# mjmj531/isaacgym

Measured on AMD Instinct MI355X. Metric: env-steps/sec at N_envs=16384 (1/2/4/8 GPUs) + achieved HBM GB/s vs roofline, higher is better.
Workload: dtype f32; 1 GPU; humanoid_pingpong 3-actor tilt (HumanoidPingpongTiltG1), num_envs=16384 per GPU, random U(-1,1) actions, 2 physics substeps per step, fused step kernel; variant=TT, kind=step, num_envs_per_gpu=16384, global_envs=16384, horizon_stats_every=32, prewarm_launches=512, full=False, launch=HIP graph of 32 steps, replayed, parallelism=env-shard x1, no data-path collective

## Files before the change

__graft_entry__.py:

```python
import os
import sys

ROOT = os.path.dirname(os.path.abspath(__file__))
if ROOT not in sys.path:
    sys.path.insert(0, ROOT)


def build():
    from isaacgym_amd import _lib
    _lib.build(force=False)
    from oracle import binding as oracle_binding
    oracle_binding.build()
    sys.path.insert(0, os.path.join(ROOT, "tests"))
    import shim_binding
    shim_binding.lib()
    import dr_shim_binding
    dr_shim_binding.lib()
    import play_shim_binding
    play_shim_binding.lib()
    import play_pair_shim_binding
    play_pair_shim_binding.lib()
    import play_act_shim_binding
    play_act_shim_binding.lib()
    import play_delay_shim_binding
    play_delay_shim_binding.lib()
    import train_delay_shim_binding
    train_delay_shim_binding.lib()
    import ppo_meter_shim_binding
    ppo_meter_shim_binding.lib()
    import render_shim_binding
    render_shim_binding.lib()
    import render_aa_shim_binding
    render_aa_shim_binding.lib()
    import ta_outcome_shim_binding
    ta_outcome_shim_binding.lib()
    import serve_shim_binding
    serve_shim_binding.lib()
    import serve_curric_shim_binding
    serve_curric_shim_binding.lib()
    import urdf_assets
    urdf_assets.build_second_arm_library()
    urdf_assets.build_second_ta_library()
    import isaacgym_amd
    L = _lib.lib()
    from isaacgym_amd import scene
    assert L.ppenv_abi_version() == scene.ABI_VERSION


def smoke():
    import numpy as np
    import torch
    from isaacgym_amd import _lib, scene
    from isaacgym_amd.env import PPEnv
    from oracle import binding as oracle_binding
    sys.path.insert(0, os.path.join(ROOT, "tests"))
    import helpers

    assert torch.cuda.is_available(), "smoke() needs the GPU box"
    _lib.lib()
    n = 256
    cfg = scene.build_config("TT", num_envs=n, seed=1)
    env = PPEnv(scene.build_config("TT", num_envs=n, seed=1), device="cuda:0")
    ora = oracle_binding.OracleEnv(cfg)
    probe = helpers.SensitivityProbe(oracle_binding, cfg)
    oa, ra = helpers.obs_atol(), helpers.reward_atol(cfg)
    rng = np.random.default_rng(0)
    excluded = 0
    for t in range(8):
        a = rng.uniform(-1, 1, (n, 7)).astype(np.float32)
        st = ora.get_state()
        env.set_state(st)
        ora.step(a)
        env.step(torch.from_numpy(a).cuda())
        torch.cuda.synchronize()
        keep = ~probe.sensitive(st, a, ora)
        excluded += int((~keep).sum())
        assert np.array_equal(env.reset_buf.cpu().numpy()[keep], ora.reset_buf[keep])
        helpers.assert_close(env.obs_buf.cpu().numpy()[keep], ora.obs_buf[keep], f"smoke: obs, step {t}", atol=oa)
        helpers.assert_close(env.rew_buf.cpu().numpy()[keep], ora.rew_buf[keep], f"smoke: rew, step {t}", atol=ra)
    assert excluded <= 4, excluded
    assert env.status == 0
    env.close()
    print(f"smoke ok: fused HIP step matches the CPU oracle on {n} envs x 8 steps (rtol 1e-4, the tests' atol; {excluded} env-steps on a switch set aside)")


if __name__ == "__main__":
    build()
    if len(sys.argv) > 1 and sys.argv[1] == "smoke":
        smoke()
```

isaacgym_amd/csrc/ppenv.hip:

```cpp
#include <hip/hip_runtime.h>

#include <algorithm>
#include <cstdio>
#include <cstdlib>
#include <cstring>
#include <new>

using std::min;
using std::max;

#if defined(PP_STAMP)
__device__ unsigned long long pp_stamp_buf[4096 * 32];
#endif
#include "ppenv_device.h"
#include "ppenv_host.h"

using namespace pp;

namespace {

constexpr int kBlock = 64;
constexpr int kObsStride = PPENV_NUM_OBS + 1;
constexpr int kMaxSplitSubsteps = 4;

// ... 354 lines not shown
        return;
    }

    PP_STAMP_AT(16);
    constexpr int EB = kBlock / BW;
    const int bw = wave - A;
    const int env = bw * EB + lane;
    const int bi = base + env;
    const bool bactive = lane < EB && bi < n;
    EnvStateT<A> st;
    float rew[A], pre_vx = 0.f;
    long long reset = 0;
    V3 next_serve = mk(0, 0, 0);
    ArmGeom<T::kShapes> g[A];
    V3 bound[A];
    float qs[A * ND], qds[A * ND];
    EnvDR bdr;
    uint32_t bdr_ep0 = 0;
#pragma unroll
    for (int a = 0; a < A; a++) rew[a] = 0.f;
    if (bactive) {
        if (!G) {
#pragma unroll
            for (int d = 0; d < A * ND; d++) { qs[d] = b.dof_pos[(size_t)d * n + bi]; qds[d] = b.dof_vel[(size_t)d * n + bi]; }
        }
        float bl[13];
#pragma unroll
        for (int k = 0; k < 13; k++) bl[k] = b.ball[(size_t)k * n + bi];
        st.ball.p = mk(bl[0], bl[1], bl[2]);
#pragma unroll
        for (int k = 0; k < 4; k++) st.ball.quat[k] = bl[3 + k];
        st.ball.v = mk(bl[7], bl[8], bl[9]);
        st.ball.w = mk(bl[10], bl[11], bl[12]);
        st.progress = b.progress[(size_t)bi * A];
#pragma unroll
        for (int a = 0; a < A; a++) st.flags[a] = b.flags[(size_t)a * n + bi];
        st.episode = b.episode[bi];
        pre_vx = st.ball.v.x;
#pragma unroll
        for (int a = 0; a < A; a++) { static_geometry<T>(K.site[a], g[a]); bound[a] = ld3(K.site[a].bound_center); }
        if (DR) {
            bdr.es = drt.es ? drt.es[bi] : 1.f;
            bdr.fs = drt.fs ? drt.fs[bi] : 1.f;
            bdr.obs_sigma = drt.obs_sigma;
            bdr.key_progress = (uint32_t)st.progress;
            bdr_ep0 = st.episode;
        }
    }
    PP_STAMP_AT(17);
    for (int s = 0; s < substeps; s++) {
        if (G) {
#pragma unroll
            for (int a = 0; a < A; a++) PP_AWAIT(&s_gflag[a], s + 1);
        } else if (s > 0) {
#pragma unroll
            for (int a = 0; a < A; a++) PP_AWAIT(&s_flag[a], s);
            if (bactive) {
#pragma unroll
                for (int a = 0; a < A; a++)
#pragma unroll
                    for (int d = 0; d < ND; d++) { qs[a * ND + d] = s_q[s - 1][a * 2 * ND + d][env]; qds[a * ND + d] = s_q[s - 1][a * 2 * ND + ND + d][env]; }
            }
        }
        PP_STAMP_AT(18 + 2 * s);
        if (bactive) {
#pragma unroll
            for (int a = 0; a < A; a++) {
                if (G) {
                    MovingGeom<T>::each(g[a], [&](int k, float& v) { v = s_geom[s & 1][a][k][env]; });
                } else {
                    JointSave js[ND];
                    GeomVisitor<T> gv(g[a]);
                    fk_sweep<T>(K.site[a], &qs[a * ND], &qds[a * ND], js, gv);
                }
            }
            PP_STAMP_AT(25);
            ball_substep<T, A, DR>(K, st.ball, g, bound, &bdr);
        }
        if (G) publish(&s_bflag, s + 1);
        PP_STAMP_AT(19 + 2 * s);
    }
#pragma unroll
    for (int a = 0; a < A; a++) PP_AWAIT(&s_flag[a], substeps + 1);
    if (bactive) {
        BodyState bodies[A * NB];
        LdsRowStore stores[A];
#pragma unroll
        for (int a = 0; a < A; a++) {
#pragma unroll
            for (int d = 0; d < ND; d++) {
                st.q[a * ND + d] = s_q[substeps - 1][a * 2 * ND + d][env];
                st.qd[a * ND + d] = s_q[substeps - 1][a * 2 * ND + ND + d][env];
                st.dof_force[a * ND + d] = s_tau[a * ND + d][env];
            }
            static_body<false>(K.site[a], bodies[a * NB]);
            bodies[a * NB + NB - 1].pos = mk(s_paddle[a * 3 + 0][env], s_paddle[a * 3 + 1][env], s_paddle[a * 3 + 2][env]);
            stores[a].row = &s_obs[(a * kBlock + env) * kObsStride];
        }
        next_serve = mk(s_serve[0][env], s_serve[1][env], s_serve[2][env]);
        if (DR && drt.obs_sigma > 0.f) {
            NoisyRowStore nstores[A];
#pragma unroll
            for (int a = 0; a < A; a++)
                nstores[a] = NoisyRowStore{stores[a].row, bdr.obs_sigma, K.seed, (uint32_t)(K.env_id_offset + bi), bdr_ep0, bdr.key_progress, 16u + (uint32_t)(a * PPENV_NUM_OBS)};
            post_physics_env<A, false>(K, (uint32_t)(K.env_id_offset + bi), st, bodies, pre_vx, &next_serve, rew, reset, nstores);
        } else
            post_physics_env<A, false>(K, (uint32_t)(K.env_id_offset + bi), st, bodies, pre_vx, &next_serve, rew, reset, stores);
        s_reset[env] = (int)reset;
    }
    publish(&s_flag_ball, 1);
    PP_STAMP_AT(22);
    __builtin_amdgcn_wave_barrier();
    PP_STAMP_AT(23);
#pragma unroll
    for (int a = 0; a < A; a++)
        flush_obs_cols<6 * NB, PPENV_NUM_OBS>(s_obs, b.obs, a * kBlock + bw * EB, BW == 1 ? nvalid : max(0, min(EB, nvalid - bw * EB)),
                                              (size_t)(base + bw * EB) * A + a, A, lane);
    if (bactive) {
        if (kBallStoresDofs) {
#pragma unroll
            for (int d = 0; d < A * ND; d++) {
                st_state(&b.dof_pos[(size_t)d * n + bi], st.q[d]);
                st_state(&b.dof_vel[(size_t)d * n + bi], st.qd[d]);
                st_state(&b.dof_force[(size_t)d * n + bi], st.dof_force[d]);
            }
        }
        store_ball(b, n, bi, st.ball);
        store_task<A>(b, n, bi, st, rew, reset);
    }
    PP_STAMP_AT(24);
}

template <class T, int A>
__global__ __launch_bounds__(kBlock) void init_kernel(const StepConsts K, DevBuffers b, int mode, int serve_on) {
    __shared__ float s_obs[A * kBlock * kObsStride];
    const int n = K.num_envs;
    const int base = blockIdx.x * kBlock;
    const int lane = threadIdx.x;
    const int i = base + lane;
    const int nvalid = min(kBlock, n - base);
    if (i < n) {
        EnvStateT<A> st;
        st.episode = mode == 0 ? 0u : b.episode[i] + 1u;
        V3 serve = serve_on ? mk(b.serve[i], b.serve[(size_t)n + i], b.serve[2 * (size_t)n + i])
                            : serve_velocity(K, (uint32_t)(K.env_id_offset + i), st.episode);
        reset_state(K, st, serve, true);
#pragma unroll
        for (int d = 0; d < A * ND; d++) st.dof_force[d] = 0.f;
        st.progress = 0;
        float rew[A];
#pragma unroll
        for (int a = 0; a < A; a++) {
            st.flags[a] = PPENV_FLAG_NO_BOUNCE;
            rew[a] = 0.f;
            BodyState bodies[NB];
            bodies_of_state<T>(K.site[a], &st.q[a * ND], &st.qd[a * ND], bodies);
            V3 bpos[NB], bvel[NB];
#pragma unroll
            for (int j = 0; j < NB; j++) { bpos[j] = bodies[j].pos; bvel[j] = bodies[j].lin; }
            LdsRowStore store{&s_obs[(a * kBlock + lane) * kObsStride]};
            write_obs(bpos, bvel, K.site[a].hinv, &st.q[a * ND], &st.qd[a * ND], st.ball.p, st.ball.v, store);
        }
        store_state<A>(b, n, i, st, rew, 1);
    }
    __syncthreads();
#pragma unroll
// ... 662 lines not shown
```

isaacgym_amd/csrc/ppenv_device.h:

```cpp
#pragma once

#include <math.h>
#include <stddef.h>
#include <stdint.h>
#include <string.h>

#include "../../include/ppenv.h"

#if defined(__HIPCC__)
#define PP_HD __host__ __device__ __forceinline__
#else
#define PP_HD inline __attribute__((always_inline))
#endif

#if defined(PP_STAMP) && defined(__HIP_DEVICE_COMPILE__)
#define PP_STAMP_AT(k)                                                                      \
    do {                                                                                    \
        __builtin_amdgcn_sched_barrier(0);                                                  \
        unsigned long long t_;                                                              \
        asm volatile("s_memtime %0\n\ts_waitcnt lgkmcnt(0)" : "=s"(t_) : : "memory");      \
        __builtin_amdgcn_sched_barrier(0);                                                  \
        if ((threadIdx.x & 63) == 0) pp_stamp_buf[blockIdx.x * 32 + (k)] = t_;                      \
    } while (0)
extern __device__ unsigned long long pp_stamp_buf[];
// ... 224 lines not shown
    float sa, ca, sz, cz;
    sincos_small(tilt_deg * deg, sa, ca);
    sincos_small(tilt_z_deg * deg, sz, cz);
    if (form == PPENV_VARIANT_T3) return mk(-speed * ca, -speed * sa, 0.f);
    if (form == PPENV_VARIANT_TT || form == PPENV_VARIANT_T4) return mk(-speed * ca * cz, -speed * sa * sz, -speed * sa);
    return mk(-speed * ca * cz, speed * sa * cz, speed * sz);
}
PP_HD V3 serve_velocity(const StepConsts& K, uint32_t gid, uint32_t episode) {
    float u0 = rng_uniform(K.seed, gid, episode, 0);
    float u1 = rng_uniform(K.seed, gid, episode, 1);
    float u2 = rng_uniform(K.seed, gid, episode, 2);
    float speed = K.serve_speed_lo + (K.serve_speed_hi - K.serve_speed_lo) * u0;
    float a = K.serve_tilt_lo_deg + (K.serve_tilt_hi_deg - K.serve_tilt_lo_deg) * u1;
    float az = K.serve_tilt_z_lo_deg + (K.serve_tilt_z_hi_deg - K.serve_tilt_z_lo_deg) * u2;
    return serve_from_draws(K.rc.variant, speed, a, az);
}
PP_HD float pd_target(float action, float lo, float hi, float clip) {
    const float a = fminf(fmaxf(action, -clip), clip);
    return 0.5f * (hi + lo) + 0.5f * (hi - lo) * a;
}

struct EnvDR {
    float kp[PPENV_NUM_DOF], kd[PPENV_NUM_DOF], ms[PPENV_NUM_DOF];
    float es, fs;
    float act_sigma, obs_sigma;
    uint32_t key_progress;
};
PP_HD void dr_gauss_pair(uint64_t seed, uint32_t gid, uint32_t episode, uint32_t progress, uint32_t pair, float& g_cos, float& g_sin) {
    const uint32_t k = progress * 256u + 2u * pair;
    const float u1 = rng_uniform(seed ^ 0x5DEECE66Dull, gid, episode, 2u * k), u2 = rng_uniform(seed ^ 0x5DEECE66Dull, gid, episode, 2u * k + 1u);
#if defined(__HIP_DEVICE_COMPILE__)
    const float rad = __builtin_amdgcn_sqrtf(-1.3862944f * __builtin_amdgcn_logf(fmaxf(u1, 5.9604645e-8f)));
    g_cos = rad * __builtin_amdgcn_cosf(u2);
    g_sin = rad * __builtin_amdgcn_sinf(u2);
#else
    const float rad = sqrtf(-2.0f * logf(fmaxf(u1, 5.9604645e-8f)));
    g_cos = rad * cosf(6.2831853f * u2);
    g_sin = rad * sinf(6.2831853f * u2);
#endif
}
PP_HD float dr_gauss(uint64_t seed, uint32_t gid, uint32_t episode, uint32_t progress, uint32_t index) {
    float c, s;
    dr_gauss_pair(seed, gid, episode, progress, index >> 1, c, s);
    return (index & 1u) ? s : c;
}

struct JointKin { float origin_xyz[3]; float origin_rot[9]; };
struct JointDrive { float lower, upper, kp, kd, effort, vel_limit, armature; };
struct JointInertial { float mass; float com[3]; float inertia[6]; };
struct ModelShape { float a[3], b[3]; float radius; };
struct ModelPaddle { float center[3], normal[3]; float radius, half_thickness; };


template <int NSHAPES>
struct ArmGeom {
    V3 pc, pn, vpc, pnd;
    V3 a[NSHAPES], b[NSHAPES];
    V3 va[NSHAPES], vb[NSHAPES];
};

struct JointSave {
    float c, s;
    V3 w, v;
    V3 ua, ub;
    float dinv, u;
};

struct BodyState { V3 pos; M3 rot; V3 lin, ang; };

template <class T, class Visitor>
PP_HD void fk_sweep(const ArmSite& S, const float* q, const float* qd, JointSave* js, Visitor& vis) {
    M3 Rp = ldm(S.base_rot);
    V3 pp = ld3(S.base_pos);
    V3 wp = mk(0, 0, 0), vp = mk(0, 0, 0);
#pragma unroll
    for (int i = 0; i < ND; i++) {
        const JointKin J = T::kin(i);
        float s, c;
        sincos_joint(q[i], s, c);
        M3 E = T::axis(i) == 0 ? joint_rot<0>(J.origin_rot, c, s) : (T::axis(i) == 1 ? joint_rot<1>(J.origin_rot, c, s) : joint_rot<2>(J.origin_rot, c, s));
        V3 r = ld3(J.origin_xyz);
        V3 pw = pp + mul(Rp, r);
        M3 Rw = mul(Rp, E);
        V3 w = tmul(E, wp);
        V3 v = tmul(E, vp + cross(wp, r));
        if (T::axis(i) == 0) w.x += qd[i]; else if (T::axis(i) == 1) w.y += qd[i]; else w.z += qd[i];
        js[i].c = c; js[i].s = s; js[i].w = w; js[i].v = v;
        vis(i, Rw, pw, w, v);
        Rp = Rw; pp = pw; wp = w; vp = v;
    }
}

template <class T>
struct GeomVisitor {
    ArmGeom<T::kShapes>& g;
    PP_HD explicit GeomVisitor(ArmGeom<T::kShapes>& gg) : g(gg) {}
    PP_HD void operator()(int i, const M3& Rw, V3 pw, V3 w, V3 v) {
        const V3 ww = mul(Rw, w), vw = mul(Rw, v);
        if (i == ND - 1) {
            const ModelPaddle P = T::paddle();
            V3 off = mul(Rw, ld3(P.center));
            g.pc = pw + off;
            g.vpc = vw + cross(ww, off);
            g.pn = mul(Rw, ld3(P.normal));
            g.pnd = cross(ww, g.pn);
        }
#pragma unroll
        for (int s = 0; s < T::kShapes; s++)
            if (T::shape_link(s) == i) {
                const ModelShape sh = T::shape(s);
                V3 oa = mul(Rw, ld3(sh.a)), ob = mul(Rw, ld3(sh.b));
                g.a[s] = pw + oa; g.va[s] = vw + cross(ww, oa);
                g.b[s] = pw + ob; g.vb[s] = vw + cross(ww, ob);
            }
    }
};
template <class T>
PP_HD void static_geometry(const ArmSite& S, ArmGeom<T::kShapes>& g) {
#pragma unroll
    for (int s = 0; s < T::kShapes; s++)
        if (T::shape_link(s) < 0) { g.a[s] = ld3(S.static_a[s]); g.b[s] = ld3(S.static_b[s]); g.va[s] = mk(0, 0, 0); g.vb[s] = mk(0, 0, 0); }
}

template <class T, bool FULL>
struct BodyVisitor {
    ArmGeom<T::kShapes>& g;
    BodyState* bodies;
    PP_HD BodyVisitor(ArmGeom<T::kShapes>& gg, BodyState* b) : g(gg), bodies(b) {}
    PP_HD void operator()(int i, const M3& Rw, V3 pw, V3 w, V3 v) {
        GeomVisitor<T> gv(g);
        gv(i, Rw, pw, w, v);
        V3 ww = mul(Rw, w), vw = mul(Rw, v);
        bodies[1 + i].pos = pw; bodies[1 + i].lin = vw;
        if (FULL) { bodies[1 + i].rot = Rw; bodies[1 + i].ang = ww; }
        if (i == ND - 1) {
#pragma unroll
            for (int j = 8; j < NB; j++) {
                const JointKin f = T::tip_frame(j);
                V3 off = mul(Rw, ld3(f.origin_xyz));
                bodies[j].pos = pw + off;
                bodies[j].lin = vw + cross(ww, off);
                if (FULL) { bodies[j].rot = mul(Rw, ldm(f.origin_rot)); bodies[j].ang = ww; }
            }
        }
    }
};
template <bool FULL>
PP_HD void static_body(const ArmSite& S, BodyState& b) {
    b.pos = ld3(S.root_pos); b.lin = mk(0, 0, 0);
    if (FULL) { b.rot = ldm(S.root_rot); b.ang = mk(0, 0, 0); }
}

template <class T, bool DR = false>
PP_HD void aba_solve(const ArmSite& S, JointSave* js, const float* qd, const float* tau, const float* arm_eff, float* qdd, const EnvDR* dr = nullptr) {
    S3 cA = {0, 0, 0, 0, 0, 0}, cD = {0, 0, 0, 0, 0, 0};
    M3 cB = {{0, 0, 0, 0, 0, 0, 0, 0, 0}};
    V3 cn = mk(0, 0, 0), cf = mk(0, 0, 0);
#pragma unroll
    for (int i = ND - 1; i >= 0; i--) {
        const JointKin JK = T::kin(i);
        const JointInertial J = T::inertial(i);
        const int ax = T::axis(i);
        V3 w = js[i].w, v = js[i].v;
        const float msc = DR ? dr->ms[i] : 1.f;
        float m = DR ? J.mass * msc : J.mass;
        V3 cm = ld3(J.com);
        V3 mc = cm * m;
        float cc = dot(cm, cm);
        float Jin[6];
#pragma unroll
        for (int t = 0; t < 6; t++) Jin[t] = DR ? J.inertia[t] * msc : J.inertia[t];
        S3 A = {Jin[0] + m * (cc - cm.x * cm.x), Jin[1] + m * (cc - cm.y * cm.y), Jin[2] + m * (cc - cm.z * cm.z),
                Jin[3] - m * cm.x * cm.y, Jin[4] - m * cm.x * cm.z, Jin[5] - m * cm.y * cm.z};
        V3 h_ang = mul(A, w) + cross(mc, v);
        V3 h_lin = v * m - cross(mc, w);
        V3 pn = cross(w, h_ang) + cross(v, h_lin) + cn;
        V3 pf = cross(w, h_lin) + cf;
        add_sym(A, cA);
        M3 B = {{cB.m[0], cB.m[1] - mc.z, cB.m[2] + mc.y, cB.m[3] + mc.z, cB.m[4], cB.m[5] - mc.x, cB.m[6] - mc.y, cB.m[7] + mc.x, cB.m[8]}};
        S3 D = {cD.xx + m, cD.yy + m, cD.zz + m, cD.xy, cD.xz, cD.yz};

        V3 ua = symcol(A, ax), ub = row(B, ax);
        float dinv = rcp_fast(symdiag(A, ax) + arm_eff[i]);
        float u = tau[i] - comp(pn, ax);
        js[i].ua = ua; js[i].ub = ub; js[i].dinv = dinv; js[i].u = u;
        if (i > 0) {
            sym_rank1_sub(A, ua, dinv);
            sym_rank1_sub(D, ub, dinv);
            V3 uad = ua * dinv;
#pragma unroll
            for (int r = 0; r < 3; r++) {
                float k = comp(uad, r);
                B.m[3 * r] -= k * ub.x; B.m[3 * r + 1] -= k * ub.y; B.m[3 * r + 2] -= k * ub.z;
            }
            V3 e = unit(ax);
            V3 cw = cross(w, e) * qd[i], cv = cross(v, e) * qd[i];
            float ud = u * dinv;
            V3 pan = pn + mul(A, cw) + mul(B, cv) + ua * ud;
            V3 paf = pf + tmul(B, cw) + mul(D, cv) + ub * ud;
            M3 E = ax == 0 ? joint_rot<0>(JK.origin_rot, js[i].c, js[i].s) : (ax == 1 ? joint_rot<1>(JK.origin_rot, js[i].c, js[i].s) : joint_rot<2>(JK.origin_rot, js[i].c, js[i].s));
            V3 r = ld3(JK.origin_xyz);
            S3 Ar = rot_sym(E, A), Dr = rot_sym(E, D);
            M3 Br = mul_t(mul(E, B), E);
            V3 nr = mul(E, pan), fr = mul(E, paf);
            M3 Dm = from_sym(Dr);
            M3 Bp;
#pragma unroll
            for (int j = 0; j < 3; j++) {
                V3 x = cross(r, col(Dm, j));
                Bp.m[j] = Br.m[j] + x.x; Bp.m[3 + j] = Br.m[3 + j] + x.y; Bp.m[6 + j] = Br.m[6 + j] + x.z;
            }
            V3 wp0 = cross(r, row(Bp, 0)), wp1 = cross(r, row(Bp, 1)), wp2 = cross(r, row(Bp, 2));
            V3 wb0 = cross(r, row(Br, 0)), wb1 = cross(r, row(Br, 1)), wb2 = cross(r, row(Br, 2));
            cA.xx = Ar.xx + wp0.x + wb0.x; cA.yy = Ar.yy + wp1.y + wb1.y; cA.zz = Ar.zz + wp2.z + wb2.z;
            cA.xy = Ar.xy + wp1.x + wb0.y; cA.xz = Ar.xz + wp2.x + wb0.z; cA.yz = Ar.yz + wp2.y + wb1.z;
            cB = Bp; cD = Dr;
            cn = nr + cross(r, fr); cf = fr;
        }
    }
    V3 aw = mk(0, 0, 0);
    V3 av = ld3(S.base_grav);
#pragma unroll
    for (int i = 0; i < ND; i++) {
        const JointKin J = T::kin(i);
        const int ax = T::axis(i);
        M3 E = ax == 0 ? joint_rot<0>(J.origin_rot, js[i].c, js[i].s) : (ax == 1 ? joint_rot<1>(J.origin_rot, js[i].c, js[i].s) : joint_rot<2>(J.origin_rot, js[i].c, js[i].s));
        V3 r = ld3(J.origin_xyz);
        V3 e = unit(ax);
        V3 aw2 = tmul(E, aw) + cross(js[i].w, e) * qd[i];
        V3 av2 = tmul(E, av + cross(aw, r)) + cross(js[i].v, e) * qd[i];
        float a = (js[i].u - dot(js[i].ua, aw2) - dot(js[i].ub, av2)) * js[i].dinv;
        qdd[i] = a;
        if (ax == 0) aw2.x += a; else if (ax == 1) aw2.y += a; else aw2.z += a;
        aw = aw2; av = av2;
    }
}

template <class T, bool DR = false>
PP_HD void arm_substep(const ArmSite& S, JointSave* js, float* q, float* qd, const float* target, float h, float* tau_drive, const EnvDR* dr = nullptr) {
    float tau[ND], arm[ND], qdd[ND];
#pragma unroll
    for (int d = 0; d < ND; d++) {
        const JointDrive J = T::drive(d);
        const float kp = DR ? J.kp * dr->kp[d] : J.kp, kd = DR ? J.kd * dr->kd[d] : J.kd;
        float err = target[d] - q[d];
        tau[d] = fminf(fmaxf(kp * (err - h * qd[d]) - kd * qd[d], -J.effort), J.effort);
        arm[d] = J.armature + h * kd + h * h * kp;
    }
    aba_solve<T, DR>(S, js, qd, tau, arm, qdd, dr);
#pragma unroll
    for (int d = 0; d < ND; d++) {
        const JointDrive J = T::drive(d);
        const float kp = DR ? J.kp * dr->kp[d] : J.kp, kd = DR ? J.kd * dr->kd[d] : J.kd;
        float err = target[d] - q[d];
        float vn = qd[d] + h * qdd[d];
        tau_drive[d] = fminf(fmaxf(kp * (err - h * vn) - kd * vn, -J.effort), J.effort);
        vn = fminf(fmaxf(vn, -J.vel_limit), J.vel_limit);
        float qn = q[d] + h * vn;
        if (qn > J.upper) { qn = J.upper; vn = fminf(vn, 0.f); }
        if (qn < J.lower) { qn = J.lower; vn = fmaxf(vn, 0.f); }
        q[d] = qn; qd[d] = vn;
    }
}

struct Ball { V3 p, v, w; float quat[4]; };

struct BallConsts {
    float contact_offset, bounce_threshold, depen_cap, r;
    float inv_kr;
    float stick_factor;
};

PP_HD void contact_resolve(const BallConsts& k, Ball& b, V3 n, float s, V3 u, float e, float mu) {
    if (!(s < k.contact_offset)) return;
    V3 vrel = b.v + cross(b.w, n * (-k.r)) - u;
    float vn = dot(vrel, n);
    if (vn < 0.f) {
        float e_eff = (-vn > k.bounce_threshold) ? e : 0.f;
        float jn = -(1.f + e_eff) * vn;
        V3 vt = vrel - n * vn;
        float vt2 = dot(vt, vt);
        if (vt2 > 1e-18f) {
            float inv = rsq_fast(vt2);
            V3 dir = vt * inv;
            float jt = fminf(mu * jn, vt2 * inv * k.stick_factor);
            b.v = b.v - dir * jt;
            b.w = b.w + cross(n, dir) * (jt * k.inv_kr);
        }
        b.v = b.v + n * jn;
    }
    if (s < 0.f) b.p = madd(b.p, n, fminf(-s, k.depen_cap));
}
PP_HD float clampf(float x, float lo, float hi) { return fminf(fmaxf(x, lo), hi); }

PP_HD void contact_box(const BallConsts& k, Ball& b, const ppenv_box& box) {
    V3 d = b.p - ld3(box.center);
    V3 h = ld3(box.half);
    float reach = k.r + k.contact_offset;
// ... 80 lines not shown
    V3 sc0[A][T::kShapes], svc[A][T::kShapes];
    float sr2[A][T::kShapes];
#pragma unroll
    for (int arm = 0; arm < A; arm++)
#pragma unroll
        for (int s = 0; s < T::kShapes; s++) {
            sc0[arm][s] = (g[arm].a[s] + g[arm].b[s]) * 0.5f;
            svc[arm][s] = (g[arm].va[s] + g[arm].vb[s]) * 0.5f;
            V3 hl = (g[arm].b[s] - g[arm].a[s]) * 0.5f;
            float rr = sqrtf(dot(hl, hl)) + T::shape(s).radius + reach;
            sr2[arm][s] = rr * rr;
        }
    PP_STAMP_AT(26);
    for (int m = 0; m < M; m++) {
        const float t = (float)m * hb;
        PP_STAMP_AT(27 + (m & 3));
        b.v.z += gdv;
        b.w = b.w * damp;
        contact_resolve(k, b, mk(0, 0, 1), b.p.z - ground_z - k.r, mk(0, 0, 0), ground_e, ground_mu);
        contact_box(k, b, table);
        contact_box(k, b, net);
#pragma unroll
        for (int arm = 0; arm < A; arm++) {
            const ArmGeom<T::kShapes>& ga = g[arm];
            V3 db = b.p - bound[arm];
            if (dot(db, db) < K.bound_r2) {
                V3 cc = madd(ga.pc, ga.vpc, t);
                V3 dpc = b.p - cc;
                if (dot(dpc, dpc) < pad_r2) {
                    V3 nn = madd(ga.pn, ga.pnd, t);
                    nn = nn * rsq_fast(dot(nn, nn));
                    contact_disc(k, b, cc, nn, ga.vpc, ga.pnd, P.radius, P.half_thickness, pad_e, pad_mu);
                }
#pragma unroll
                for (int s = 0; s < T::kShapes; s++) {
                    V3 dsc = b.p - madd(sc0[arm][s], svc[arm][s], t);
                    if (dot(dsc, dsc) < sr2[arm][s]) {
                        const float radius = T::shape(s).radius;
                        const float e = DR ? fminf(K.shape_e[s] * dr->es, e_cap) : K.shape_e[s], mu = DR ? K.shape_mu[s] * dr->fs : K.shape_mu[s];
                        if (T::shape_link(s) < 0)
                            contact_capsule(k, b, ga.a[s], ga.b[s], mk(0, 0, 0), mk(0, 0, 0), radius, e, mu);
                        else
                            contact_capsule(k, b, madd(ga.a[s], ga.va[s], t), madd(ga.b[s], ga.vb[s], t), ga.va[s], ga.vb[s], radius, e, mu);
                    }
                }
            }
        }
        b.p = madd(b.p, b.v, hb);
    }
    PP_STAMP_AT(31);
    float wx = b.w.x, wy = b.w.y, wz = b.w.z, x = b.quat[0], y = b.quat[1], z = b.quat[2], w = b.quat[3];
    float kq = 0.5f * h;
    float nx = x + kq * (wx * w + wy * z - wz * y);
    float ny = y + kq * (wy * w + wz * x - wx * z);
    float nz = z + kq * (wz * w + wx * y - wy * x);
    float nw = w + kq * (-wx * x - wy * y - wz * z);
    float inv = rsq_fast(nx * nx + ny * ny + nz * nz + nw * nw);
    b.quat[0] = nx * inv; b.quat[1] = ny * inv; b.quat[2] = nz * inv; b.quat[3] = nw * inv;
}

PP_HD V3 quat_rotate(const float q[4], V3 v) {
    float qw = q[3];
    V3 qv = mk(q[0], q[1], q[2]);
    float s = 2.0f * (qw * qw) - 1.0f;
    V3 cr = cross(qv, v);
    float d = dot(qv, v);
    return mk(v.x * s + cr.x * qw * 2.0f + qv.x * d * 2.0f, v.y * s + cr.y * qw * 2.0f + qv.y * d * 2.0f,
              v.z * s + cr.z * qw * 2.0f + qv.z * d * 2.0f);
}
PP_HD void heading_quat_inv(const float q[4], float out[4]) {
    V3 rd = quat_rotate(q, mk(1, 0, 0));
    float heading = atan2f(rd.y, rd.x);
    float theta = (-heading) / 2.0f;
    float sz = sinf(theta), w = cosf(theta);
    float nrm = fmaxf(sqrtf(sz * sz + w * w), 1e-9f);
    out[0] = 0.f; out[1] = 0.f; out[2] = sz / nrm; out[3] = w / nrm;
}

PP_HD V3 heading_rotate(const float hinv[4], V3 v) {
    float qw = hinv[3], sz = hinv[2];
    float s = 2.0f * (qw * qw) - 1.0f;
    float k = sz * qw * 2.0f;
    return mk(v.x * s - v.y * k, v.y * s + v.x * k, v.z);
}

struct RewardIn {
    float humanoid_x;
    V3 paddle;
    float pre_vx;
    V3 bp;
    float vx;
    float power;
    long long progress;
};

PP_HD float compute_reward(const RewardConsts& c, const RewardIn& in, uint32_t& flags, long long& reset) {
    const float Bx = in.bp.x, By = in.bp.y, Bz = in.bp.z, vx = in.vx, pre_vx = in.pre_vx;
    const float alpha = c.alpha, penalty = c.penalty, threshold = 0.1f;
    const float power_reward = -c.power_coefficient * in.power;
    const int variant = c.variant;
    uint32_t f = flags;
    float reward;
    long long die = 0;
    if (variant == PPENV_VARIANT_T3) {
        V3 dp = in.paddle - in.bp;
        float dist = sqrtf(dp.x * dp.x + dp.y * dp.y + dp.z * dp.z);
        float pos_reward = 1.0f / (1.0f + 1.5f * dist * dist);
        float vel_reward = (pre_vx < 0.f && vx > 0.f) ? alpha * fabsf(vx) : 0.f;
        reward = pos_reward + power_reward + vel_reward;
        bool missed = Bx < in.paddle.x - 1e-3f;
        if (missed) { reward = reward + penalty; die = 1; }
        if (Bz < threshold) die = 1;
    } else if (variant == PPENV_VARIANT_TT || variant == PPENV_VARIANT_T4) {
        V3 dp = in.paddle - in.bp;
        float dist = sqrtf(dp.x * dp.x + dp.y * dp.y + dp.z * dp.z);
        float pos_reward = 1.0f / (1.0f + 1.5f * dist * dist);
        bool cond = pre_vx < 0.f && vx > 0.f;
        float vel_reward = (cond && !(f & PPENV_FLAG_COND_CALC)) ? alpha * fabsf(vx) : 0.f;
        if (cond) f |= PPENV_FLAG_COND_CALC;
        bool missed = Bx < in.humanoid_x - 0.05f;
        reward = missed ? 0.f + penalty : 0.f;
        bool bounce = Bz < 0.83f && vx > 0.f && By < 0.6f && By > -0.6f;
        float hit = 0.f;
        bool early = Bx < 2.44f && bounce;
        if (early && !(f & PPENV_FLAG_REWARD_CALC)) hit = c.not_hit_table_penalty;
        if (early) { f |= PPENV_FLAG_REWARD_CALC; f &= ~PPENV_FLAG_NO_BOUNCE; }
        bool inx = Bx > 2.44f && Bx < 3.1f;
        bool good = inx && bounce && (f & PPENV_FLAG_NO_BOUNCE);
        if (good && !(f & PPENV_FLAG_REWARD_CALC)) hit = c.hit_table_reward;
        if (good) f |= PPENV_FLAG_REWARD_CALC;
        if (Bx >= 3.1f && vx > 0.f && !(f & PPENV_FLAG_REWARD_CALC)) hit = c.not_hit_table_penalty;
        if (Bx >= 3.1f) f |= PPENV_FLAG_REWARD_CALC;
        float net = (Bx > 1.7f && Bx < 1.8f && vx > 0.f && By < 0.4f && By > -0.4f && Bz > 0.98f && Bz < 1.14f) ? 400.f : 0.f;
        reward += (((pos_reward + power_reward) + vel_reward) + hit) + net;
        if (Bz < threshold) die = 1;
    } else {
        bool hit_paddle = pre_vx < 0.f && vx > 1.0f;
        bool missed = (Bx < in.humanoid_x - 0.05f) || (Bx < in.paddle.x - 0.1f);
        reward = (!(f & PPENV_FLAG_MISSED_CALC) && missed) ? 0.f + penalty : 0.f;
        if (missed) f |= PPENV_FLAG_MISSED_CALC;
        float dy = in.paddle.y - By, dz = in.paddle.z - Bz;
        float dist = sqrtf(dy * dy + dz * dz);
        float pos_reward = 0.f;
        if (!(f & PPENV_FLAG_COND_CALC) || (Bx < in.humanoid_x - 0.05f)) pos_reward = 1.0f * expf(-20.0f * dist * dist);
        float vel_reward = (hit_paddle && !(f & PPENV_FLAG_COND_CALC)) ? alpha * fabsf(vx) : 0.f;
        if (hit_paddle) f |= PPENV_FLAG_COND_CALC;
        reward += (pos_reward + power_reward) + vel_reward;
        if (Bz < threshold) reward = -800.f + reward;
    }
    flags = f;
    reset = (in.progress >= (long long)c.max_episode_length - 1) ? 1 : die;
    return reward;
}

PP_HD float compute_reward_side2(const RewardConsts& c, const RewardIn& in, uint32_t& flags, long long& reset) {
    const float Bx = in.bp.x, By = in.bp.y, Bz = in.bp.z, vx = in.vx, pre_vx = in.pre_vx;
    uint32_t f = flags;
    V3 dp = in.paddle - in.bp;
    float dist = sqrtf(dp.x * dp.x + dp.y * dp.y + dp.z * dp.z);
    float pos_reward = 1.0f / (1.0f + 1.5f * dist * dist);
    bool cond = pre_vx > 0.f && vx < 0.f;
    float vel_reward = (cond && !(f & PPENV_FLAG_COND_CALC)) ? c.alpha * fabsf(vx) : 0.f;
    if (cond) f |= PPENV_FLAG_COND_CALC;
    bool missed = Bx > in.humanoid_x + 0.05f;
    float reward = missed ? 0.f + c.penalty : 0.f;
    bool bounce = Bz < 0.83f && vx < 0.f && By < 0.6f && By > -0.6f;
// ... 17 lines not shown

template <int A>
struct EnvStateT {
    float q[A * ND], qd[A * ND], dof_force[A * ND];
    Ball ball;
    long long progress;
    uint32_t flags[A], episode;
};
using EnvState = EnvStateT<1>;

template <class T, int A, bool DR = false>
PP_HD void simulate_env(const StepConsts& K, const float* actions, EnvStateT<A>& st, BodyState* bodies, float& pre_vx, const EnvDR* dr = nullptr, uint32_t gid = 0) {
    float target[A * ND];
#pragma unroll
    for (int d = 0; d < A * ND; d++) {
        float act = actions[d];
        if (DR) { if (dr->act_sigma > 0.f) act += dr->act_sigma * dr_gauss(K.seed, gid, st.episode, dr->key_progress, (uint32_t)d); }
        target[d] = pd_target(act, T::drive(d % ND).lower, T::drive(d % ND).upper, K.clip_actions);
    }
    pre_vx = st.ball.v.x;
    const int substeps = K.substeps;
    const float h = K.h;
    JointSave js[A][ND];
    ArmGeom<T::kShapes> g[A];
    V3 bound[A];
#pragma unroll
    for (int a = 0; a < A; a++) {
        bound[a] = ld3(K.site[a].bound_center);
        static_geometry<T>(K.site[a], g[a]);
        GeomVisitor<T> gv(g[a]);
        fk_sweep<T>(K.site[a], &st.q[a * ND], &st.qd[a * ND], js[a], gv);
    }
    PP_STAMP_AT(2);
    for (int s = 0; s < substeps; s++) {
        ball_substep<T, A, DR>(K, st.ball, g, bound, dr);
        PP_STAMP_AT(3 + 3 * s);
#pragma unroll
        for (int a = 0; a < A; a++)
            arm_substep<T, DR>(K.site[a], js[a], &st.q[a * ND], &st.qd[a * ND], &target[a * ND], h, &st.dof_force[a * ND], dr);
        PP_STAMP_AT(4 + 3 * s);
#pragma unroll
        for (int a = 0; a < A; a++) {
            if (s + 1 < substeps) {
                GeomVisitor<T> gv(g[a]);
                fk_sweep<T>(K.site[a], &st.q[a * ND], &st.qd[a * ND], js[a], gv);
            } else {
                BodyVisitor<T, false> bv(g[a], &bodies[a * NB]);
                fk_sweep<T>(K.site[a], &st.q[a * ND], &st.qd[a * ND], js[a], bv);
            }
        }
        PP_STAMP_AT(5 + 3 * s);
    }
#pragma unroll
    for (int a = 0; a < A; a++) static_body<false>(K.site[a], bodies[a * NB]);
}

template <class T>
PP_HD void bodies_of_state(const ArmSite& S, const float* q, const float* qd, BodyState* bodies) {
    JointSave js[ND];
    ArmGeom<T::kShapes> g;
    BodyVisitor<T, true> bv(g, bodies);
    fk_sweep<T>(S, q, qd, js, bv);
    static_body<true>(S, bodies[0]);
}

template <int A>
PP_HD void reset_state(const StepConsts& K, EnvStateT<A>& st, V3 serve, bool reset_dofs) {
    st.ball.p = ld3(K.ball_init_pos);
#pragma unroll
    for (int k = 0; k < 4; k++) st.ball.quat[k] = K.ball_init_quat[k];
    st.ball.v = serve;
    st.ball.w = mk(0, 0, 0);
    if (reset_dofs) {
#pragma unroll
        for (int d = 0; d < A * ND; d++) { st.q[d] = K.init_dof_pos[d % ND]; st.qd[d] = K.init_dof_vel[d % ND]; }
    }
}

template <int J0 = 0, int J1 = NB, class Store>
PP_HD void write_obs_bodies(const V3* body_pos, const V3* body_vel, const float hinv[4], Store& store) {
    V3 root = body_pos[0];
#pragma unroll
    for (int j = J0; j < J1; j++) {
        V3 lp = heading_rotate(hinv, body_pos[j] - root);
        V3 lv = heading_rotate(hinv, body_vel[j]);
        store(3 * j, lp.x); store(3 * j + 1, lp.y); store(3 * j + 2, lp.z);
        store(3 * NB + 3 * j, lv.x); store(3 * NB + 3 * j + 1, lv.y); store(3 * NB + 3 * j + 2, lv.z);
    }
}
template <class Store>
PP_HD void write_obs_tail(V3 root, const float hinv[4], const float* q, const float* qd, V3 ball_p, V3 ball_v, Store& store) {
#pragma unroll
    for (int d = 0; d < ND; d++) {
        store(6 * NB + d, q[d]);
        store(6 * NB + ND + d, qd[d] * 0.1f);
    }
    V3 lb = heading_rotate(hinv, ball_p - root);
    V3 lbv = heading_rotate(hinv, ball_v);
    store(6 * NB + 2 * ND, lb.x); store(6 * NB + 2 * ND + 1, lb.y); store(6 * NB + 2 * ND + 2, lb.z);
    store(6 * NB + 2 * ND + 3, lbv.x); store(6 * NB + 2 * ND + 4, lbv.y); store(6 * NB + 2 * ND + 5, lbv.z);
}
template <class Store>
PP_HD void write_obs(const V3* body_pos, const V3* body_vel, const float hinv[4], const float* q, const float* qd,
                     V3 ball_p, V3 ball_v, Store& store) {
    write_obs_bodies(body_pos, body_vel, hinv, store);
    write_obs_tail(body_pos[0], hinv, q, qd, ball_p, ball_v, store);
}

template <int A, bool BODY_OBS = true, class Store>
PP_HD void post_physics_env(const StepConsts& K, uint32_t gid, EnvStateT<A>& st, const BodyState* bodies, float pre_vx,
                            const V3* serve_override, float* rew, long long& reset, Store* stores) {
    st.progress += 1;
    RewardIn in;
    in.humanoid_x = K.site[0].root_pos[0];
    in.paddle = bodies[NB - 1].pos;
    in.pre_vx = pre_vx;
    in.bp = st.ball.p;
    in.vx = st.ball.v.x;
    float power = 0.f;
#pragma unroll
    for (int d = 0; d < A * ND; d++) power += fabsf(st.dof_force[d] * st.qd[d]);
    in.power = power;
    in.progress = st.progress;
    rew[0] = compute_reward(K.rc, in, st.flags[0], reset);
    if (A > 1) {
        RewardIn in2 = in;
        in2.humanoid_x = K.site[A - 1].root_pos[0];
        in2.paddle = bodies[(A - 1) * NB + NB - 1].pos;
        long long reset2;
        rew[A - 1] = compute_reward_side2(K.rc, in2, st.flags[A - 1], reset2);
        reset = (reset | reset2) ? 1 : 0;
    }
    if (reset) {
        st.episode += 1;
        V3 serve = serve_override ? *serve_override : serve_velocity(K, gid, st.episode);
        reset_state(K, st, serve, K.rc.variant != PPENV_VARIANT_TN);
        st.progress = 0;
#pragma unroll
        for (int a = 0; a < A; a++) st.flags[a] = PPENV_FLAG_NO_BOUNCE;
    }
#pragma unroll
    for (int a = 0; a < A; a++) {
        if (BODY_OBS) {
            V3 bpos[NB], bvel[NB];
#pragma unroll
            for (int j = 0; j < NB; j++) { bpos[j] = bodies[a * NB + j].pos; bvel[j] = bodies[a * NB + j].lin; }
            write_obs_bodies(bpos, bvel, K.site[a].hinv, stores[a]);
        }
        write_obs_tail(bodies[a * NB].pos, K.site[a].hinv, &st.q[a * ND], &st.qd[a * ND], st.ball.p, st.ball.v, stores[a]);
    }
}

}

namespace pp {
inline RewardConsts make_reward_consts(const ppenv_config& c) {
    RewardConsts r;
    r.variant = c.variant; r.max_episode_length = c.max_episode_length;
    r.alpha = c.alpha_velocity_reward; r.power_coefficient = c.power_coefficient; r.penalty = c.penalty;
    r.hit_table_reward = c.hit_table_reward; r.not_hit_table_penalty = c.not_hit_table_penalty;
    return r;
}
inline StepConsts make_step_consts(const ppenv_config& c) {
    StepConsts K;
    memset(&K, 0, sizeof K);
    K.num_envs = c.num_envs; K.env_id_offset = c.env_id_offset; K.substeps = c.substeps; K.ball_substeps = c.ball_substeps;
    K.num_arms = c.num_humanoids == 2 ? 2 : 1;
    K.seed = c.seed;
// ... 100 lines not shown
```

Before: 1.433 billion env-steps/s.

## Pack paired 3-vector ops into two-lane types across FK, ABA and obs

Introduces packed pair operations (V3p/S3p) so twin rotations, cross products and rank-1 updates in forward kinematics, the articulated-body solve and observation heading rotation run together. The aim is to let the compiler emit packed two-wide f32 math (e.g. v_pk_fma_f32 on CDNA) and cut instruction count in the ALU-bound step kernel. It also skips the geometry visitor for links that carry no collision shapes, and adds a timing stamp point. This risks higher register pressure and small FP rounding differences. Contraction is disabled in the inertia helper to keep it matching the oracle.

```diff
diff --git a/__graft_entry__.py b/__graft_entry__.py
--- a/__graft_entry__.py
+++ b/__graft_entry__.py
@@ -38,6 +38,8 @@
     serve_shim_binding.lib()
     import serve_curric_shim_binding
     serve_curric_shim_binding.lib()
+    import packed_pairs_shim_binding
+    packed_pairs_shim_binding.lib()
     import urdf_assets
     urdf_assets.build_second_arm_library()
     urdf_assets.build_second_ta_library()
diff --git a/isaacgym_amd/csrc/ppenv.hip b/isaacgym_amd/csrc/ppenv.hip
--- a/isaacgym_amd/csrc/ppenv.hip
+++ b/isaacgym_amd/csrc/ppenv.hip
@@ -460,6 +460,7 @@
     }
 #pragma unroll
     for (int a = 0; a < A; a++) PP_AWAIT(&s_flag[a], substeps + 1);
+    PP_STAMP_AT(11);
     if (bactive) {
         BodyState bodies[A * NB];
         LdsRowStore stores[A];
diff --git a/isaacgym_amd/csrc/ppenv_device.h b/isaacgym_amd/csrc/ppenv_device.h
--- a/isaacgym_amd/csrc/ppenv_device.h
+++ b/isaacgym_amd/csrc/ppenv_device.h
@@ -330,8 +330,8 @@
         V3 r = ld3(J.origin_xyz);
         V3 pw = pp + mul(Rp, r);
         M3 Rw = mul(Rp, E);
-        V3 w = tmul(E, wp);
-        V3 v = tmul(E, vp + cross(wp, r));
+        V3p wv = tmul(E, pk(wp, vp + cross(wp, r)));
+        V3 w = lo(wv), v = hi(wv);
         if (T::axis(i) == 0) w.x += qd[i]; else if (T::axis(i) == 1) w.y += qd[i]; else w.z += qd[i];
         js[i].c = c; js[i].s = s; js[i].w = w; js[i].v = v;
         vis(i, Rw, pw, w, v);
@@ -344,22 +344,30 @@
     ArmGeom<T::kShapes>& g;
     PP_HD explicit GeomVisitor(ArmGeom<T::kShapes>& gg) : g(gg) {}
     PP_HD void operator()(int i, const M3& Rw, V3 pw, V3 w, V3 v) {
-        const V3 ww = mul(Rw, w), vw = mul(Rw, v);
+        bool used = i == ND - 1;
+#pragma unroll
+        for (int s = 0; s < T::kShapes; s++) used = used || T::shape_link(s) == i;
+        if (!used) return;
+        const V3p wv = mul(Rw, pk(w, v));
+        const V3 ww = lo(wv), vw = hi(wv);
         if (i == ND - 1) {
             const ModelPaddle P = T::paddle();
-            V3 off = mul(Rw, ld3(P.center));
+            const V3p on = mul(Rw, pk(ld3(P.center), ld3(P.normal)));
+            const V3 off = lo(on);
+            const V3p x = cross(ww, on);
             g.pc = pw + off;
-            g.vpc = vw + cross(ww, off);
-            g.pn = mul(Rw, ld3(P.normal));
-            g.pnd = cross(ww, g.pn);
+            g.vpc = vw + lo(x);
+            g.pn = hi(on);
+            g.pnd = hi(x);
         }
 #pragma unroll
         for (int s = 0; s < T::kShapes; s++)
             if (T::shape_link(s) == i) {
                 const ModelShape sh = T::shape(s);
-                V3 oa = mul(Rw, ld3(sh.a)), ob = mul(Rw, ld3(sh.b));
-                g.a[s] = pw + oa; g.va[s] = vw + cross(ww, oa);
-                g.b[s] = pw + ob; g.vb[s] = vw + cross(ww, ob);
+                const V3p o = mul(Rw, pk(ld3(sh.a), ld3(sh.b)));
+                const V3p x = cross(ww, o);
+                g.a[s] = pw + lo(o); g.va[s] = vw + lo(x);
+                g.b[s] = pw + hi(o); g.vb[s] = vw + hi(x);
             }
     }
 };
@@ -378,17 +386,20 @@
     PP_HD void operator()(int i, const M3& Rw, V3 pw, V3 w, V3 v) {
         GeomVisitor<T> gv(g);
         gv(i, Rw, pw, w, v);
-        V3 ww = mul(Rw, w), vw = mul(Rw, v);
+        const V3p wv = mul(Rw, pk(w, v));
+        const V3 ww = lo(wv), vw = hi(wv);
         bodies[1 + i].pos = pw; bodies[1 + i].lin = vw;
         if (FULL) { bodies[1 + i].rot = Rw; bodies[1 + i].ang = ww; }
         if (i == ND - 1) {
-#pragma unroll
-            for (int j = 8; j < NB; j++) {
-                const JointKin f = T::tip_frame(j);
-                V3 off = mul(Rw, ld3(f.origin_xyz));
-                bodies[j].pos = pw + off;
-                bodies[j].lin = vw + cross(ww, off);
-                if (FULL) { bodies[j].rot = mul(Rw, ldm(f.origin_rot)); bodies[j].ang = ww; }
+            static_assert(NB == 10, "the two bodies that ride on the last link are handled as a pair");
+            const JointKin f8 = T::tip_frame(8), f9 = T::tip_frame(9);
+            const V3p off = mul(Rw, pk(ld3(f8.origin_xyz), ld3(f9.origin_xyz)));
+            const V3p x = cross(ww, off);
+            bodies[8].pos = pw + lo(off); bodies[8].lin = vw + lo(x);
+            bodies[9].pos = pw + hi(off); bodies[9].lin = vw + hi(x);
+            if (FULL) {
+                bodies[8].rot = mul(Rw, ldm(f8.origin_rot)); bodies[8].ang = ww;
+                bodies[9].rot = mul(Rw, ldm(f9.origin_rot)); bodies[9].ang = ww;
             }
         }
     }
@@ -399,6 +410,23 @@
     if (FULL) { b.rot = ldm(S.root_rot); b.ang = mk(0, 0, 0); }
 }
 
+template <bool DR>
+PP_HD void link_inertia(const JointInertial& J, float msc, float& m, V3& mc, S3& A) {
+#if defined(__clang__)
+#pragma clang fp contract(off)
+#endif
+    m = DR ? J.mass * msc : J.mass;
+    V3 cm = ld3(J.com);
+    mc = cm * m;
+    float cc = dot(cm, cm);
+    float Jin[6];
+#pragma unroll
+    for (int t = 0; t < 6; t++) Jin[t] = DR ? J.inertia[t] * msc : J.inertia[t];
+    S3 a = {Jin[0] + m * (cc - cm.x * cm.x), Jin[1] + m * (cc - cm.y * cm.y), Jin[2] + m * (cc - cm.z * cm.z),
+            Jin[3] - m * cm.x * cm.y, Jin[4] - m * cm.x * cm.z, Jin[5] - m * cm.y * cm.z};
+    A = a;
+}
+
 template <class T, bool DR = false>
 PP_HD void aba_solve(const ArmSite& S, JointSave* js, const float* qd, const float* tau, const float* arm_eff, float* qdd, const EnvDR* dr = nullptr) {
     S3 cA = {0, 0, 0, 0, 0, 0}, cD = {0, 0, 0, 0, 0, 0};
@@ -410,20 +438,15 @@
         const JointInertial J = T::inertial(i);
         const int ax = T::axis(i);
         V3 w = js[i].w, v = js[i].v;
-        const float msc = DR ? dr->ms[i] : 1.f;
-        float m = DR ? J.mass * msc : J.mass;
-        V3 cm = ld3(J.com);
-        V3 mc = cm * m;
-        float cc = dot(cm, cm);
-        float Jin[6];
-#pragma unroll
-        for (int t = 0; t < 6; t++) Jin[t] = DR ? J.inertia[t] * msc : J.inertia[t];
-        S3 A = {Jin[0] + m * (cc - cm.x * cm.x), Jin[1] + m * (cc - cm.y * cm.y), Jin[2] + m * (cc - cm.z * cm.z),
-                Jin[3] - m * cm.x * cm.y, Jin[4] - m * cm.x * cm.z, Jin[5] - m * cm.y * cm.z};
+        float m;
+        V3 mc;
+        S3 A;
+        link_inertia<DR>(J, DR ? dr->ms[i] : 1.f, m, mc, A);
         V3 h_ang = mul(A, w) + cross(mc, v);
         V3 h_lin = v * m - cross(mc, w);
-        V3 pn = cross(w, h_ang) + cross(v, h_lin) + cn;
-        V3 pf = cross(w, h_lin) + cf;
+        V3p wxh = cross(w, pk(h_ang, h_lin));
+        V3 pn = lo(wxh) + cross(v, h_lin) + cn;
+        V3 pf = hi(wxh) + cf;
         add_sym(A, cA);
         M3 B = {{cB.m[0], cB.m[1] - mc.z, cB.m[2] + mc.y, cB.m[3] + mc.z, cB.m[4], cB.m[5] - mc.x, cB.m[6] - mc.y, cB.m[7] + mc.x, cB.m[8]}};
         S3 D = {cD.xx + m, cD.yy + m, cD.zz + m, cD.xy, cD.xz, cD.yz};
@@ -433,8 +456,9 @@
         float u = tau[i] - comp(pn, ax);
         js[i].ua = ua; js[i].ub = ub; js[i].dinv = dinv; js[i].u = u;
         if (i > 0) {
-            sym_rank1_sub(A, ua, dinv);
-            sym_rank1_sub(D, ub, dinv);
+            S3p AD = pk(A, D);
+            const V3p uab = pk(ua, ub);
+            sym_rank1_sub(AD, uab, dinv);
             V3 uad = ua * dinv;
 #pragma unroll
             for (int r = 0; r < 3; r++) {
@@ -442,15 +466,17 @@
                 B.m[3 * r] -= k * ub.x; B.m[3 * r + 1] -= k * ub.y; B.m[3 * r + 2] -= k * ub.z;
             }
             V3 e = unit(ax);
-            V3 cw = cross(w, e) * qd[i], cv = cross(v, e) * qd[i];
+            V3p c = cross(pk(w, v), e) * qd[i];
+            V3 cw = lo(c), cv = hi(c);
             float ud = u * dinv;
-            V3 pan = pn + mul(A, cw) + mul(B, cv) + ua * ud;
-            V3 paf = pf + tmul(B, cw) + mul(D, cv) + ub * ud;
+            V3p pa = pk(pn, pf) + mul(AD, c) + pk(mul(B, cv), tmul(B, cw)) + uab * ud;
             M3 E = ax == 0 ? joint_rot<0>(JK.origin_rot, js[i].c, js[i].s) : (ax == 1 ? joint_rot<1>(JK.origin_rot, js[i].c, js[i].s) : joint_rot<2>(JK.origin_rot, js[i].c, js[i].s));
             V3 r = ld3(JK.origin_xyz);
-            S3 Ar = rot_sym(E, A), Dr = rot_sym(E, D);
+            const S3p ADr = rot_sym(E, AD);
+            const S3 Ar = lo(ADr), Dr = hi(ADr);
             M3 Br = mul_t(mul(E, B), E);
-            V3 nr = mul(E, pan), fr = mul(E, paf);
+            const V3p nfr = mul(E, pa);
+            V3 nr = lo(nfr), fr = hi(nfr);
             M3 Dm = from_sym(Dr);
             M3 Bp;
 #pragma unroll
@@ -458,10 +484,9 @@
                 V3 x = cross(r, col(Dm, j));
                 Bp.m[j] = Br.m[j] + x.x; Bp.m[3 + j] = Br.m[3 + j] + x.y; Bp.m[6 + j] = Br.m[6 + j] + x.z;
             }
-            V3 wp0 = cross(r, row(Bp, 0)), wp1 = cross(r, row(Bp, 1)), wp2 = cross(r, row(Bp, 2));
-            V3 wb0 = cross(r, row(Br, 0)), wb1 = cross(r, row(Br, 1)), wb2 = cross(r, row(Br, 2));
-            cA.xx = Ar.xx + wp0.x + wb0.x; cA.yy = Ar.yy + wp1.y + wb1.y; cA.zz = Ar.zz + wp2.z + wb2.z;
-            cA.xy = Ar.xy + wp1.x + wb0.y; cA.xz = Ar.xz + wp2.x + wb0.z; cA.yz = Ar.yz + wp2.y + wb1.z;
+            V3p w0 = cross(r, pk(row(Bp, 0), row(Br, 0))), w1 = cross(r, pk(row(Bp, 1), row(Br, 1))), w2 = cross(r, pk(row(Bp, 2), row(Br, 2)));
+            cA.xx = Ar.xx + w0.x[0] + w0.x[1]; cA.yy = Ar.yy + w1.y[0] + w1.y[1]; cA.zz = Ar.zz + w2.z[0] + w2.z[1];
+            cA.xy = Ar.xy + w1.x[0] + w0.y[1]; cA.xz = Ar.xz + w2.x[0] + w0.z[1]; cA.yz = Ar.yz + w2.y[0] + w1.z[1];
             cB = Bp; cD = Dr;
             cn = nr + cross(r, fr); cf = fr;
         }
@@ -708,6 +733,13 @@
     float s = 2.0f * (qw * qw) - 1.0f;
     float k = sz * qw * 2.0f;
     return mk(v.x * s - v.y * k, v.y * s + v.x * k, v.z);
+}
+PP_HD V3p heading_rotate(const float hinv[4], V3p v) {
+    float qw = hinv[3], sz = hinv[2];
+    float s = 2.0f * (qw * qw) - 1.0f;
+    float k = sz * qw * 2.0f;
+    V3p r = {v.x * s - v.y * k, v.y * s + v.x * k, v.z};
+    return r;
 }
 
 struct RewardIn {
@@ -891,8 +923,8 @@
     V3 root = body_pos[0];
 #pragma unroll
     for (int j = J0; j < J1; j++) {
-        V3 lp = heading_rotate(hinv, body_pos[j] - root);
-        V3 lv = heading_rotate(hinv, body_vel[j]);
+        const V3p l = heading_rotate(hinv, pk(body_pos[j] - root, body_vel[j]));
+        const V3 lp = lo(l), lv = hi(l);
         store(3 * j, lp.x); store(3 * j + 1, lp.y); store(3 * j + 2, lp.z);
         store(3 * NB + 3 * j, lv.x); store(3 * NB + 3 * j + 1, lv.y); store(3 * NB + 3 * j + 2, lv.z);
     }
```

Result: faster. 1.454 billion env-steps/s (median of 6 runs) (+1.4%).
